# google/sentencepiece

Hardware: AMD Instinct MI355X
Metric: sentences/sec EncodeBatch, 32k unigram, MI355X (higher is better)
Workload: dtype u8 text -> i32 ids; f64 add / f32 store in the Viterbi relax

## Files before the change

### sentencepiece_amd/csrc/api.cc

```cpp
#include <hip/hip_runtime.h>

#include <cstdio>
#include <cstdlib>
#include <fcntl.h>
#include <sys/mman.h>
#include <sys/stat.h>
#include <sys/syscall.h>
#include <unistd.h>

#include <algorithm>
#include <cmath>
#include <condition_variable>
#include <cstring>
#include <fstream>
#include <functional>
#include <map>
#include <memory>
#include <mutex>
#include <thread>
#include <new>
#include <sstream>
#include <atomic>
#include <chrono>
#include <string>
// ... 135 lines not shown
      auto it = live.find(p);
      if (it == live.end()) return false;
      const size_t cap = it->second;
      live.erase(it);
      if (idle_bytes + cap > (24ull << 30)) drop = p;
      else { idle.emplace(cap, p); idle_bytes += cap; }
    }
    if (drop) (void)hipHostFree(drop);
    return true;
  }
};
PinnedPool g_pinned;

struct Profile {
  int n = 0;
  char name[kNumSlots][48] = {{0}};
  float kernel_ms[kNumSlots] = {0};
  uint64_t sentences[kNumSlots] = {0}, raw_bytes[kNumSlots] = {0}, ids[kNumSlots] = {0};
  uint64_t cycles[kNumSlots][5] = {{0}};
  uint64_t path[8] = {0};
  float total_ms = 0.f;
};

struct Workspace {
  DevBuf<uint32_t> d_lists, d_counts;
  DevBuf<uint64_t> d_tmp_off, d_tile_sums, d_chunk_base;
  DevBuf<uint32_t> d_big_list;
  DevBuf<int32_t> d_arena, d_arena_tb, d_tok_begin;
  DevBuf<uint32_t> d_span_begin, d_span_end, d_nspan_begin, d_nspan_end;
  DevBuf<uint8_t> d_norm, d_nbest_scratch, d_slab, d_pool, d_sent_status, d_flags;
  DevBuf<unsigned long long> d_res_off, d_dyn_tag;
  DevBuf<U4> d_dyn_ent, d_resume;
  DevBuf<uint32_t> d_dyn_list;
  DevBuf<float> d_res_score;
  Ctrl *d_ctrl = nullptr;
  Ctrl *h_ctrl = nullptr;
  DevBuf<uint8_t> d_text, d_dn_text;
  DevBuf<uint64_t> d_offs, d_id_offs, d_dn_offs;
  DevBuf<int32_t> d_ids;
  DevBuf<uint8_t> d_lit_bytes;
  DevBuf<uint32_t> d_lit_offs;
  DevBuf<int32_t> d_dec_ids;
  DevBuf<uint64_t> d_dec_poffs;
  const uint8_t *lit_bytes = nullptr;
  const uint32_t *lit_offs = nullptr;
  uint32_t n_lit = 0;
  PinBuf<uint8_t> h_text;
  PinBuf<uint64_t> h_offs, h_id_offs;
  uint64_t reserve_text_bytes = 0, reserve_n = 0;
  float bpe_dropout = 0.f;
  uint64_t sample_seed = 0;
  hipStream_t stream = nullptr;
  hipStream_t stream2 = nullptr;
  hipEvent_t ev_fork = nullptr, ev_join = nullptr;
  hipEvent_t ev[kNumSlots + 1][2] = {};
  bool ev_ready = false;
  bool slot_used[kNumSlots] = {false};
  char slot_name[kNumSlots][48] = {{0}};
  Profile prof;

  ~Workspace() {
    d_lists.Free(); d_counts.Free(); d_tmp_off.Free(); d_tile_sums.Free(); d_chunk_base.Free(); d_big_list.Free(); d_arena.Free();
    d_arena_tb.Free(); d_tok_begin.Free(); d_span_begin.Free(); d_span_end.Free(); d_nspan_begin.Free(); d_nspan_end.Free();
    d_norm.Free(); d_nbest_scratch.Free(); d_slab.Free(); d_pool.Free(); d_sent_status.Free(); d_flags.Free(); d_res_off.Free();
    d_res_score.Free(); d_dyn_tag.Free(); d_dyn_ent.Free(); d_dyn_list.Free(); d_resume.Free(); d_text.Free(); d_offs.Free(); d_id_offs.Free(); d_ids.Free(); d_dn_text.Free(); d_dn_offs.Free();
    h_text.Free(); h_offs.Free(); h_id_offs.Free();
// ... 27 lines not shown
  }
};
}
using spmx_tables::DevTables;

struct spmx_handle : DevTables {
  std::mutex mu;
  ModelData model;
  HostTables tables;
  std::string extra_options;
  std::string serialized;
  int device = 0;
  int n_cu = 256;
  SpmxDev dev{};
  HostTables dn_tables;
  DevBuf<uint32_t> dn_ndarts, dn_npair;
  DevBuf<uint8_t> dn_nblob;
  DevBuf<U2> dn_utrie;
  SpmxDev dn_dev{};
  std::vector<std::unique_ptr<Workspace>> pool;
  bool profiling = false;
  Profile prof;
  bool no_fast = false;
  bool no_lane_general = false;
  uint32_t char_norm_mode = 0;
  bool no_stream = false;
  uint64_t arena_first = 0;
  bool no_bp_short = false;
  bool no_wave = false;
  std::atomic<int> word_backoff{0};
  bool no_word = false;
  bool no_word_dp = false;
  uint32_t dyn_slots = kDynSlotsDefault;
  uint32_t dyn_list_cap = kDynListCapDefault;
  uint64_t nbest_budget = 32ull << 30;
  uint32_t nbest_hyps_min = 4096;
  uint32_t tile_min_lanes = 1;
  int32_t dx_npre = 0, dx_nsuf = 0, dx_pre[kMaxExtra] = {0}, dx_suf[kMaxExtra] = {0};
  bool dx_reverse = false;
  bool dx_unk = false;
  uint32_t compact_staged = 2048;
  bool no_direct = false;
  int fork_cus = 0;
  int fork_waves = 4;
  bool early_tail = false;
  bool no_overlap = false;
  bool no_ids16 = false;
  bool no_scan = false;
  bool no_word_dyn = false;
  bool memo_unsafe = false;
  bool force_word_dp = false;
  bool no_split = false;
  uint32_t split_min_raw = 576;
  bool split_own_launch = false;
  uint32_t split_tiles = 1;
  uint32_t split_per_byte = 4;
  uint32_t compact_big = kCompactBigIds;
  bool uw_exact = false;
  int uw_pipe = 1;
  bool no_uni_wave = false;
  uint32_t uni_wave_max = 0;
  int word_wgs = 1;
  uint64_t table_bytes = 0;
  uint64_t dn_table_bytes = 0;
  double load_ms = 0.0;
  int word_form = 3;
// ... 107 lines not shown
  dev->umemo16 = d->d_umemo16.p;
  dev->uall = d->d_uall.p;
  dev->udisp = d->d_udisp.p;
  dev->uhot2 = d->d_uhot2.p;
  dev->uhot = d->d_uhot.p;
  dev->pscore = d->d_pscore.p;
  dev->sym_final = d->d_sym_final.p;
  dev->sym_len = d->d_sym_len.p;
  dev->byte_ids = d->d_byte_ids.p;
  dev->dec_info = d->d_dec_info.p;
  dev->dec_off = d->d_dec_off.p;
  dev->dec_bytes = d->d_dec_bytes.p;
  return kOk;
}

int UploadDenormTables(spmx_handle *h) {
  if (!h->model.has_denormalizer) return kOk;
  const HostTables &d = h->dn_tables;
  HIP_OR_RETURN(h, Upload(&h->dn_ndarts, d.ndarts));
  HIP_OR_RETURN(h, Upload(&h->dn_nblob, d.nblob));
  HIP_OR_RETURN(h, Upload(&h->dn_npair, d.npair));
  HIP_OR_RETURN(h, Upload(&h->dn_utrie, d.utrie));
  h->dn_dev = d.scalars;
  h->dn_dev.ndarts = h->dn_ndarts.p;
  h->dn_dev.nblob = h->dn_nblob.p;
  h->dn_dev.npair = h->dn_npair.p;
  h->dn_dev.utrie = h->dn_utrie.p;
  return kOk;
}

int RefreshDevice(spmx_handle *h, bool types_changed) {
  HostTables &t = h->tables;
  if (types_changed) {
    if (h->model.model_type == kUnigram) {
      HIP_OR_RETURN(h, Upload(&h->d_ptrie, t.ptrie));
      HIP_OR_RETURN(h, Upload(&h->d_cfirst, t.cfirst));
    } else {
      HIP_OR_RETURN(h, Upload(&h->d_sym_final, t.sym_final));
    }
    HIP_OR_RETURN(h, Upload(&h->d_umemo, t.umemo));
    HIP_OR_RETURN(h, Upload(&h->d_umemo16, t.umemo16));
    HIP_OR_RETURN(h, Upload(&h->d_uall, t.uall));
    HIP_OR_RETURN(h, Upload(&h->d_udisp, t.udisp));
    HIP_OR_RETURN(h, Upload(&h->d_uhot2, t.uhot2));
    HIP_OR_RETURN(h, Upload(&h->d_uhot, t.uhot));
    HIP_OR_RETURN(h, Upload(&h->d_pscore, t.pscore));
    HIP_OR_RETURN(h, Upload(&h->d_dec_info, t.dec_info));
    HIP_OR_RETURN(h, Upload(&h->d_dec_off, t.dec_off));
    HIP_OR_RETURN(h, Upload(&h->d_dec_bytes, t.dec_bytes));
  }
  SpmxDev d = t.scalars;
  d.ndarts = h->dev.ndarts; d.nblob = h->dev.nblob; d.npair = h->dev.npair; d.ptrie = h->d_ptrie.p; d.cfirst = t.cfirst.empty() ? nullptr : h->d_cfirst.p; d.plen = h->d_plen.p; d.utrie = h->dev.utrie;
  d.chartab = h->dev.chartab; d.pairtab = h->dev.pairtab; d.wordtab = h->dev.wordtab; d.sym_final = h->d_sym_final.p;
  d.sym_len = h->dev.sym_len; d.byte_ids = h->dev.byte_ids;
  d.umemo = h->d_umemo.p; d.umemo16 = h->d_umemo16.p; d.uall = h->d_uall.p; d.udisp = h->d_udisp.p; d.uhot2 = h->d_uhot2.p; d.uhot = h->d_uhot.p; d.pscore = h->d_pscore.p;
  d.dec_info = h->d_dec_info.p; d.dec_off = h->d_dec_off.p; d.dec_bytes = h->d_dec_bytes.p;
  h->dev = d;
  return kOk;
}

void DestroyHandle(spmx_handle *h) {
  if (!h) return;
  (void)hipSetDevice(h->device);
  h->FreeTables();
  h->dn_ndarts.Free(); h->dn_npair.Free(); h->dn_nblob.Free(); h->dn_utrie.Free();
  h->pool.clear();
// ... 558 lines not shown
              sc.count = static_cast<uint32_t>(total);
              sc.tw = 64;
              sc.main_tiles = static_cast<uint32_t>((total + 63) / 64);
              sc.tile_base = 0;
              tile_base = sc.main_tiles;
            }
            continue;
          }
          if (known[c] == 0) continue;
          uint64_t tw = (static_cast<uint64_t>(known[c]) + n_waves - 1) / n_waves;
          if (tw > 64) tw = 64;
          if (tw < 1) tw = 1;
          sc.lane_shift = 6;
          sc.general = ((uni_class[c] && cls[c].rcap > kMaxStagedRaw) || cls[c].rcap > h->main_max_raw) ? 1u : 0u;
          sc.count = known[c];
          sc.tw = static_cast<uint32_t>(tw);
          sc.main_tiles = static_cast<uint32_t>((static_cast<uint64_t>(known[c]) + tw - 1) / tw);
          sc.tile_base = tile_base;
          tile_base += sc.main_tiles;
        }
        wa.total_main = tile_base;
        wa.q = &ws->d_ctrl->q[qi];
        wa.stats = &ws->d_ctrl->stats[kStatsPerClass * slot];
        wa.left_lists = out_lists;
        wa.left_counts = d_out_counts;
        wa.left2_lists = out2_lists;
        wa.left2_counts = d_out2_counts;
        wa.dyn_tag = ws->d_dyn_tag.p;
        wa.dyn_ent = ws->d_dyn_ent.p;
        wa.dyn_list = ws->d_dyn_list.p;
        wa.dyn_count = &ws->d_ctrl->dyn_count;
        wa.dyn_mask = h->dyn_slots - 1u;
        wa.dyn_cap = h->dyn_list_cap;
        wa.resume = ws->d_resume.p;
        wa.ids16 = ids16 ? 1u : 0u;
        wa.arena_first = (direct && mode != 2) ? direct_region : 0u;
        snprintf(ws->slot_name[slot], sizeof(ws->slot_name[slot]), "%s",
                 wform ? (wa.ids16 ? (mode == 2 ? "EncodeWordWaveAgainKernel<true>" : mode == 1 ? "EncodeWordWaveCollectKernel<true>" : "EncodeWordWaveKernel<true>")
                                   : (mode == 2 ? "EncodeWordWaveAgainKernel<false>" : mode == 1 ? "EncodeWordWaveCollectKernel<false>" : "EncodeWordWaveKernel<false>"))
                       : mode == 3 ? "EncodeWordDpKernel" : mode == 2 ? "EncodeWordAgainKernel" : mode == 1 ? "EncodeWordCollectKernel" : "EncodeWordKernel");
        HIP_OR_RETURN(h, record(slot, 0));
        if (wform) HIP_OR_RETURN(h, LaunchEncodeWordWave(mode, wa, static_cast<int>(grid), waves, WordWaveLdsBytes(waves), stream));
        else HIP_OR_RETURN(h, LaunchEncodeWord(mode, wa, static_cast<int>(grid), waves, WordLdsBytes(waves, dp), stream));
        HIP_OR_RETURN(h, record(slot, 1));
        ws->slot_used[slot] = true;
        return kOk;
      };
      auto read_counts = [&]() -> int {
        HIP_OR_RETURN(h, hipMemcpyAsync(ws->h_ctrl->left_counts, ws->d_ctrl->left_counts, sizeof(ws->h_ctrl->left_counts) + sizeof(uint32_t),
                                        hipMemcpyDeviceToHost, stream));
        HIP_OR_RETURN(h, hipStreamSynchronize(stream));
        return kOk;
      };
      uint64_t eligible = 0;
      for (int c = 0; c < ncls; ++c) if (cls[c].rcap <= h->main_max_raw) eligible += known[c];
      int left_at = 0;
      if (dyn) {
        FORKED_HIP_OR_RETURN(ws->d_dyn_tag.Reserve(h->dyn_slots));
        FORKED_HIP_OR_RETURN(ws->d_dyn_ent.Reserve(static_cast<size_t>(h->dyn_slots) * 4));
        FORKED_HIP_OR_RETURN(ws->d_dyn_list.Reserve(h->dyn_list_cap));
        FORKED_HIP_OR_RETURN(ws->d_resume.Reserve(n));
        FORKED_HIP_OR_RETURN(hipMemsetAsync(ws->d_dyn_tag.p, 0, static_cast<size_t>(h->dyn_slots) * sizeof(unsigned long long), stream));
        FORKED_OR_RETURN(word_pass(1, kSlotWord, 3, left_lists[0], ws->d_ctrl->left_counts[0], left_lists[1], ws->d_ctrl->left_counts[1]));
        FORKED_OR_RETURN(read_counts());
        for (int c = 0; c < ncls; ++c) { again_counts[c] = ws->h_ctrl->left_counts[0][c]; again_total += again_counts[c]; }
        again_words = ws->h_ctrl->dyn_count < h->dyn_list_cap ? ws->h_ctrl->dyn_count : h->dyn_list_cap;
        left_at = 1;
        if (again_total > 0) {
          uint32_t gone1[kMaxClasses] = {0};
          uint64_t gone1_total = 0;
          for (int c = 0; c < ncls; ++c) { gone1[c] = ws->h_ctrl->left_counts[1][c]; gone1_total += gone1[c]; }
          const bool early_tail = h->early_tail && direct && !forked && !h->no_overlap && gone1_total > 0;
          if (early_tail) {
            HIP_OR_RETURN(h, hipEventRecord(ws->ev_fork, stream));
            HIP_OR_RETURN(h, hipStreamWaitEvent(ws->stream2, ws->ev_fork, 0));
          }
          if (again_words) {
            ResolveArgs ra{};
            ra.dev = h->dev; ra.dyn_ent = ws->d_dyn_ent.p; ra.dyn_list = ws->d_dyn_list.p; ra.dyn_count = &ws->d_ctrl->dyn_count;
            ra.dyn_cap = h->dyn_list_cap; ra.unsafe = h->memo_unsafe ? 1u : 0u;
            uint64_t g = (static_cast<uint64_t>(again_words) + 63) / 64;
            if (g > static_cast<uint64_t>(h->n_cu) * 8) g = static_cast<uint64_t>(h->n_cu) * 8;
            FORKED_HIP_OR_RETURN(LaunchWordResolve(ra, static_cast<int>(g), stream));
          }
          if (early_tail) left_at = 2;
          for (int c = 0; c < ncls; ++c) known[c] = again_counts[c];
          a.lists = left_lists[0];
          FORKED_OR_RETURN(word_pass(2, kSlotWord2, 4, left_lists[left_at], ws->d_ctrl->left_counts[left_at], nullptr, nullptr));
          if (early_tail) {
            forked = true;
            stream = ws->stream2;
            tail_qi = 0;
            const int rc = general_pass(left_lists[1], ws->d_ctrl->left_counts[1], gone1, true);
            tail_qi = 5;
            hipError_t ej = rc == kOk ? hipEventRecord(ws->ev_join, stream) : hipSuccess;
            stream = main_stream;
            if (rc != kOk) return fail_forked(rc);
            if (ej != hipSuccess) return fail_forked(FailHip(h, ej, "hipEventRecord(join)"));
            a.lists = left_lists[0];
          }
          FORKED_OR_RETURN(read_counts());
        }
      } else {
        FORKED_OR_RETURN(word_pass(0, kSlotWord, 3, left_lists[0], ws->d_ctrl->left_counts[0], nullptr, nullptr));
        FORKED_OR_RETURN(read_counts());
        uint64_t total = 0;
        for (int c = 0; c < ncls; ++c) { known[c] = ws->h_ctrl->left_counts[0][c]; total += known[c]; }
        a.lists = left_lists[0];
        if (!is_bpe && !h->no_word_dp && total && (total * 4 <= n || h->force_word_dp)) {
          FORKED_OR_RETURN(word_pass(3, kSlotWord2, 4, left_lists[1], ws->d_ctrl->left_counts[1], nullptr, nullptr));
          FORKED_OR_RETURN(read_counts());
          left_at = 1;
        }
      }
      uint64_t leftover = 0;
      for (int c = 0; c < ncls; ++c) {
        known[c] = ws->h_ctrl->left_counts[left_at][c];
// ... 377 lines not shown
    if (st.ok()) st = CompileExtraOptions(h->model, "", &h->tables);
    if (st.ok() && h->model.has_denormalizer) {
      ModelData dn;
      dn.normalizer_only = true;
      dn.charsmap = h->model.dn_charsmap;
      dn.add_dummy_prefix = h->model.dn_add_dummy_prefix;
      dn.remove_extra_ws = h->model.dn_remove_extra_ws;
      dn.escape_ws = h->model.dn_escape_ws;
      st = CompileTables(dn, &h->dn_tables);
    }
    if (!st.ok()) return Fail(nullptr, st.code, st.message);
    HIP_OR_RETURN(nullptr, hipSetDevice(device));
    hipDeviceProp_t prop;
    HIP_OR_RETURN(nullptr, hipGetDeviceProperties(&prop, device));
    h->n_cu = prop.multiProcessorCount > 0 ? prop.multiProcessorCount : 256;
    for (int c = 0; c < kNumClasses; ++c) h->classes[c] = kClasses[c];
    if (const char *e = getenv("SPMX_NO_FAST")) h->no_fast = e[0] == '1';
    if (const char *e = getenv("SPMX_NO_STREAM")) h->no_stream = e[0] == '1';
    if (const char *e = getenv("SPMX_NO_WAVE")) h->no_wave = e[0] == '1';
    if (const char *e = getenv("SPMX_NO_WORD_KERNEL")) h->no_word = e[0] == '1';
    if (const char *e = getenv("SPMX_FORCE_WORD_DP")) h->force_word_dp = e[0] == '1';
    if (const char *e = getenv("SPMX_NO_WORD_DYN")) h->no_word_dyn = e[0] == '1';
    if (const char *e = getenv("SPMX_NO_OVERLAP")) h->no_overlap = e[0] == '1';
    if (const char *e = getenv("SPMX_EARLY_TAIL")) h->early_tail = e[0] == '1';
    if (const char *e = getenv("SPMX_FORK_WAVES")) h->fork_waves = atoi(e);
    if (const char *e = getenv("SPMX_FORK_CUS")) h->fork_cus = atoi(e);
    if (const char *e = getenv("SPMX_NO_DIRECT")) h->no_direct = e[0] == '1';
    if (const char *e = getenv("SPMX_COMPACT_STAGED")) {
      const long v = atol(e);
      h->compact_staged = v <= 0 ? 0u : v < 256 ? 256u : v > static_cast<long>(kCompactLdsIdsMax) ? kCompactLdsIdsMax : static_cast<uint32_t>(v) & ~7u;
    }
    if (const char *e = getenv("SPMX_NO_SCAN")) h->no_scan = e[0] == '1';
    if (const char *e = getenv("SPMX_NO_IDS16")) h->no_ids16 = e[0] == '1';
    if (const char *e = getenv("SPMX_DYN_SLOTS_LOG2")) { const int v = atoi(e); if (v >= 4 && v <= 26) h->dyn_slots = 1u << v; }
    if (const char *e = getenv("SPMX_DYN_LIST_CAP")) { const long v = atol(e); if (v >= 1 && v <= (1l << 26)) h->dyn_list_cap = static_cast<uint32_t>(v); }
    if (const char *e = getenv("SPMX_NBEST_BUDGET_GB")) { const long v = atol(e); if (v >= 1 && v <= 200) h->nbest_budget = static_cast<uint64_t>(v) << 30; }
#ifdef SPMX_TEST_SEAMS
    if (getenv("SPMX_WORDMEMO_UNSAFE")) h->memo_unsafe = true;
    if (getenv("SPMX_UW_EXACT")) h->uw_exact = true;
    if (const char *e = getenv("SPMX_COMPACT_BIG")) h->compact_big = static_cast<uint32_t>(atoll(e));
    if (const char *e = getenv("SPMX_NO_WORD_DP")) h->no_word_dp = e[0] == '1';
    if (const char *e = getenv("SPMX_NBEST_HYPS_MIN")) { const long v = atol(e); if (v >= 1024 && v <= 262144) h->nbest_hyps_min = static_cast<uint32_t>(v); }
    if (const char *e = getenv("SPMX_TILE_MIN_LANES")) h->tile_min_lanes = static_cast<uint32_t>(atoi(e));
    if (const char *e = getenv("SPMX_NO_UNI_WAVE")) h->no_uni_wave = e[0] == '1';
    if (const char *e = getenv("SPMX_WORD_WGS")) { const int v = atoi(e); if (v >= 1 && v <= 4) h->word_wgs = v; }
    if (const char *e = getenv("SPMX_NO_BP_SHORT")) h->no_bp_short = e[0] == '1';
    if (const char *e = getenv("SPMX_WIDE_TCAP")) h->wide_tcap = e[0] == '1';
    if (const char *e = getenv("SPMX_SUB_BUCKETS")) {
      const int v = atoi(e);
      h->sub_buckets = static_cast<uint32_t>(v < 1 ? 1 : (v > kMaxSubBuckets ? kMaxSubBuckets : v));
    }
    if (const char *e = getenv("SPMX_LANE_GENERAL_MIN_LANES")) h->lane_general_min_lanes = static_cast<uint32_t>(atoi(e));
    if (const char *e = getenv("SPMX_STREAM_SCRATCH_MB")) h->stream_scratch_limit = static_cast<uint64_t>(atoll(e)) << 20;
    if (const char *e = getenv("SPMX_MAIN_MAX_RAW")) h->main_max_raw = static_cast<uint32_t>(atoll(e));
    if (const char *e = getenv("SPMX_FORCE_RING")) { const int v = atoi(e); if (v >= 16 && v <= 122) h->ring_override = static_cast<uint32_t>(v); }
#else
    {
      static const char *const kSeamOnly[] = {"SPMX_NO_WORD_DP", "SPMX_NBEST_HYPS_MIN", "SPMX_TILE_MIN_LANES",
          "SPMX_NO_UNI_WAVE", "SPMX_WORD_WGS", "SPMX_NO_BP_SHORT", "SPMX_WIDE_TCAP", "SPMX_SUB_BUCKETS", "SPMX_LANE_GENERAL_MIN_LANES",
          "SPMX_STREAM_SCRATCH_MB", "SPMX_MAIN_MAX_RAW", "SPMX_FORCE_RING", "SPMX_MEMO16_ONE"};
      static std::atomic<bool> warned{false};
      for (const char *v : kSeamOnly)
        if (getenv(v) && !warned.exchange(true))
          fprintf(stderr, "libspmx: %s is read by test-seam builds only (-DSPMX_TEST_SEAMS); this library ignores it\n", v);
    }
#endif
// ... 112 lines not shown
    return RefreshDevice(h, true);
  });
}

namespace {

int RebuildForSpec(spmx_handle *h, bool add_dummy_prefix, bool remove_extra_ws, bool escape_ws, std::string *charsmap) {
  ModelData &m = h->model;
  struct Undo {
    ModelData &m;
    bool adp, rew, esc, done = false;
    std::string *charsmap;
    ~Undo() {
      if (done) return;
      m.add_dummy_prefix = adp; m.remove_extra_ws = rew; m.escape_ws = esc;
      if (charsmap) m.charsmap.swap(*charsmap);
    }
  } undo{m, m.add_dummy_prefix, m.remove_extra_ws, m.escape_ws, false, charsmap};
  m.add_dummy_prefix = add_dummy_prefix; m.remove_extra_ws = remove_extra_ws; m.escape_ws = escape_ws;
  if (charsmap) m.charsmap.swap(*charsmap);
  std::unique_ptr<HostTables> nt(new HostTables);
  Status st = CompileTables(m, nt.get());
  if (st.ok()) st = CompileExtraOptions(m, h->extra_options, nt.get());
  if (!st.ok()) return Fail(h, st.code, st.message);
  HIP_OR_RETURN(h, hipSetDevice(h->device));
  DevTables fresh;
  SpmxDev dev{};
  t_upload_bytes = 0;
  if (int rc = UploadTables(h, &fresh, *nt, &dev); rc != kOk) {
    fresh.FreeTables();
    return rc;
  }
  std::swap(static_cast<DevTables &>(*h), fresh);
  fresh.FreeTables();
  h->tables = std::move(*nt);
  h->dev = dev;
  h->table_bytes = t_upload_bytes + h->dn_table_bytes;
  h->word_backoff.store(0, std::memory_order_relaxed);
  undo.done = true;
  return kOk;
}

}

int spmx_override_normalizer_spec(spmx_handle *h, const char *const *fields, const char *const *values,
                                  const uint64_t *value_lens, uint64_t n) {
  if (!h) return kInvalidArgument;
  return Guard(h, [&]() -> int {
    if (n && (!fields || !values)) return Fail(h, kInvalidArgument, "null field or value array");
    std::vector<SpecEdit> edits;
    Status failed;
    for (uint64_t i = 0; i < n && failed.ok(); ++i) {
      const char *v = values[i] ? values[i] : "";
      SpecEdit e;
      failed = ParseSpecEdit(fields[i] ? fields[i] : "", std::string(v, value_lens ? value_lens[i] : strlen(v)), &e);
      if (failed.ok()) edits.push_back(std::move(e));
    }
    if (!edits.empty()) {
      bool adp = h->model.add_dummy_prefix, rew = h->model.remove_extra_ws, esc = h->model.escape_ws;
      const std::string *cm = nullptr;
      for (const SpecEdit &e : edits) {
        if (e.field == 2) cm = &e.bytes;
        else if (e.field == 3) adp = e.flag;
        else if (e.field == 4) rew = e.flag;
        else if (e.field == 5) esc = e.flag;
      }
// ... 1417 lines not shown
```

### sentencepiece_amd/csrc/kernels.h

```cpp
#ifndef SPMX_KERNELS_H_
#define SPMX_KERNELS_H_

#ifndef SPMX_WAVE_API
#include "wave.h"
#endif
#include <math.h>

#include "dev.h"

namespace spmx {

enum : uint32_t {
  kStArenaOverflow = 1u << 0,
  kStTooLong = 1u << 1,
  kStInternal = 1u << 2,
};
enum : uint32_t { kSsOk = 0, kSsResourceExhausted = 8, kSsOutOfRange = 11, kSsInternal = 13 };

constexpr int kMaxClasses = 8;

struct StreamClass {
  uint32_t rcap;
  uint32_t tcap;
  uint32_t lane_shift;
// ... 32 lines not shown
  uint8_t *sent_status;
  uint32_t *status;
  unsigned long long *stats;
  int32_t *arena_tb;
  uint32_t *long_list;
  SideLists *side;
  const uint32_t *lists;
  uint32_t *over_list;
  StreamQueue *q;
  uint8_t *slab;
  uint64_t slab_bytes;
  uint32_t n;
  uint32_t n_classes;
  uint32_t total_main;
  uint32_t bp_short;
  uint32_t ring;
  uint32_t fast_ok;
  uint32_t no_lane_general;
  uint32_t private_bytes;
  uint32_t split_ring;
  uint32_t match_rows;
  uint32_t no_char_norm;
  StreamClass cls[kMaxClasses];
  uint32_t *left_lists;
  uint32_t *left_counts;
  uint32_t *left2_lists;
  uint32_t *left2_counts;
  unsigned long long *dyn_tag;
  U4 *dyn_ent;
  uint32_t *dyn_list;
  uint32_t *dyn_count;
  uint32_t dyn_mask;
  uint32_t dyn_cap;
  U4 *resume;
  uint32_t ids16;
  uint32_t direct;
  uint64_t arena_first;
  const uint32_t *list;
  const uint32_t *list_count;
  uint32_t *next_list;
  uint32_t *next_count;
  uint32_t rcap, ncap;
};

constexpr int kStatsPerClass = 8;
constexpr uint32_t kTokEnd = 0x8000u;

SPMX_DEVICE uint32_t DartsOffset(uint32_t u) { return (u >> 10) << ((u & (1u << 9)) >> 6); }

SPMX_DEVICE int OneCharLenDev(uint32_t c) {
  const uint32_t h = c >> 4;
  return h < 12 ? 1 : (h < 14 ? 2 : (h == 14 ? 3 : 4));
}
SPMX_DEVICE uint32_t SpByteOf(const SpmxDev &d) { return (d.flags & kNfCompressSp) ? kSpByte : 0x100u; }

SPMX_DEVICE int wave_excl_scan(int v, int lane, int *total) {
  int incl = v;
#pragma unroll
  for (int d = 1; d < 64; d <<= 1) {
    const int up = wv::shfl_up(incl, d);
    if (lane >= d) incl += up;
  }
  *total = wv::shfl(incl, 63);
  return incl - v;
}

// ... 1094 lines not shown
```

### sentencepiece_amd/csrc/kernels_wordwave.h

```cpp
#ifndef SPMX_KERNELS_WORDWAVE_H_
#define SPMX_KERNELS_WORDWAVE_H_

namespace spmx {

constexpr uint32_t kWwRing = 4096u;
constexpr uint32_t kWwRingPad = 32u;
constexpr uint32_t kWwUnits = kWwRing / 16u;
constexpr uint32_t kWwMaskBytes = (kWwUnits + 4u) * 2u + 8u;
constexpr uint32_t kWwRecs = 128u + 512u;
constexpr uint32_t kWwMaxLen = 65536u;
constexpr uint32_t kWwPerWave = kWwRing + kWwRingPad + kWwMaskBytes + kWwRecs * 4u + 64u * 16u + 64u * 8u + 5u * 64u * 4u;
static_assert(kWwPerWave % 16u == 0u, "per-wave LDS blocks keep 16-byte alignment");
constexpr uint32_t kWwAgain = 1u, kWwGone = 2u;
constexpr uint32_t kWwKeyMaskBytes = 640u;
constexpr uint32_t kWwShared = kWwKeyMaskBytes + kWordHotSlots * 16u + kUallBuckets * 2u;
SPMX_HD constexpr bool kWwHotIn(int mode) { return mode == 2; }
SPMX_HD inline uint32_t WordWaveLdsBytes(uint32_t waves) { return kWwShared + waves * kWwPerWave; }

struct __attribute__((packed, aligned(2))) U64H { uint32_t lo, hi; };

SPMX_DEVICE uint32_t space_mask16(const Q4 &v) {
  auto m4 = [](uint32_t z) -> uint32_t { return (((z >> 7) & 0x01010101u) * 0x10204080u) >> 28; };
  return m4(space_flags(v.x)) | (m4(space_flags(v.y)) << 4) | (m4(space_flags(v.z)) << 8) | (m4(space_flags(v.w)) << 12);
}
SPMX_DEVICE uint32_t key_dword_n(uint32_t text, int n) {
  const uint32_t m = n >= 4 ? 0xFFFFFFFFu : (n <= 0 ? 0u : (1u << (8 * n)) - 1u);
  return key_dword(text, m);
}

struct WwStage {
  uint32_t cnt;
  uint32_t P, j;
  uint32_t L;
  uint32_t k0, k1, k2, k3;
  uint32_t hz, hw;
  uint32_t e0x, e0y, e0z, e0w, e1x, e1y, e1z, e1w;
  uint32_t tg_lo, tg_hi;
  uint32_t warm;
  uint32_t d0x, d0y, d0z, d0w, d1x, d1y, d1z, d1w, d2x, d2y, d2z, d2w;
};
constexpr uint32_t kWwHit16 = 0x100u;

template <int MODE, bool H16>
SPMX_DEVICE void encode_wordwave_block(const EncodeArgs &a, unsigned char *smem) {
  const int lane = wv::lane();
  const SpmxDev &d = a.dev;
  Q4 *masks = reinterpret_cast<Q4 *>(smem);
  U4 *hot = reinterpret_cast<U4 *>(smem + kWwKeyMaskBytes);
  uint16_t *disp = reinterpret_cast<uint16_t *>(smem + kWwKeyMaskBytes + kWordHotSlots * 16u);
// ... 158 lines not shown
    SA.cnt = 0u; SB.cnt = 0u;
    uint32_t carry_j = 0xFFFFFFFFu, carry_x = 0u, carry_n = 0u, carry_unk = 0u;
    uint32_t carry_t = 0u;
    unsigned long long steps = 0;

    auto stageA = [&](uint32_t qbase, uint32_t qcnt, WwStage &S) __attribute__((always_inline)) {
      S.cnt = qcnt;
      const uint32_t l32 = static_cast<uint32_t>(lane);
      const bool valid = l32 < qcnt;
      const uint32_t rec = recq[qbase + (valid ? l32 : (qcnt ? qcnt - 1u : 0u))];
      const uint32_t P = rec & 0x03FFFFFFu, j = rec >> 26;
      const uint32_t s_end = sent[j].y;
      const Q4U w = *reinterpret_cast<const Q4U *>(ring + (P & (kWwRing - 1u)));
      const U64H sm = *reinterpret_cast<const U64H *>(smask + ((P >> 4) & (kWwUnits - 1u)));
      const uint64_t bits = (static_cast<uint64_t>(sm.hi) << 32 | sm.lo) >> (P & 15u);
      const uint32_t rem = s_end - P;
      uint32_t L = static_cast<uint32_t>(wv::ffs64(bits | (1ull << 17))) - 1u;
      if (L > rem) L = rem;
      S.P = P; S.j = j;
      const Q4 mk = masks[2u * (L < 16u ? L : 16u)], pd = masks[2u * (L < 16u ? L : 16u) + 1u];
      S.k0 = (w.x & mk.x) | pd.x; S.k1 = (w.y & mk.y) | pd.y; S.k2 = (w.z & mk.z) | pd.z; S.k3 = (w.w & mk.w) | pd.w;
      const uint32_t h1 = HashWordKey(S.k0, S.k1, S.k2, S.k3), h2 = UallHash2(S.k0, S.k1, S.k2, S.k3, h1);
      const U4 e = kWwHotIn(MODE) ? hot[h1 & (kWordHotSlots - 1u)] : U4{0u, 0u, 0u, 0xFFFFFFFFu};
      const uint32_t dsp = disp[UallBucket(h2)];
      const uint32_t zmask = L <= 10u ? 0xFFFFu : 0xFFFFFFFFu, form = L <= 10u ? kMemo16TwoPiece : 0u;
      const bool hit16 = kWwHotIn(MODE) & (valid & (L <= 12u)) & ((e.x == S.k0) & (e.y == S.k1)) & ((((e.z ^ S.k2) & zmask) == 0u) &
                         ((e.w & kMemo16TwoPiece) == form) & (e.w != 0xFFFFFFFFu));
      S.L = L | (hit16 ? kWwHit16 : 0u);
      S.hz = e.z; S.hw = e.w;
      const uint32_t slp = perfect ? UallSlot(h1, h2, dsp, mall) : (h1 & mall);
      const uint32_t sl = (valid & !hit16 & (L <= 16u)) ? slp : 0u;
      const U4 e0 = uall[2u * sl], e1 = uall[2u * sl + 1u];
      S.e0x = e0.x; S.e0y = e0.y; S.e0z = e0.z; S.e0w = e0.w; S.e1x = e1.x; S.e1y = e1.y; S.e1z = e1.z; S.e1w = e1.w;
      if (MODE != kWmPlain) {
        const bool pre = MODE == kWmDyn || dyn_warm != 0u;
        if (MODE == kWmCollect && dyn_warm != 0u) --dyn_warm;
        const uint32_t dsl = (pre & valid & !hit16 & (L <= 16u)) ? (h1 & a.dyn_mask) : 0u;
        const unsigned long long g = MODE == kWmCollect ? wv::atomic_load64(&a.dyn_tag[dsl]) : a.dyn_tag[dsl];
        S.tg_lo = static_cast<uint32_t>(g); S.tg_hi = static_cast<uint32_t>(g >> 32);
        S.warm = pre ? 1u : 0u;
        if (MODE == kWmDyn) {
          const U4 d0 = a.dyn_ent[4u * dsl], d1 = a.dyn_ent[4u * dsl + 1u], d2 = a.dyn_ent[4u * dsl + 2u];
          S.d0x = d0.x; S.d0y = d0.y; S.d0z = d0.z; S.d0w = d0.w; S.d1x = d1.x; S.d1y = d1.y; S.d1z = d1.z; S.d1w = d1.w;
          S.d2x = d2.x; S.d2y = d2.y; S.d2z = d2.z; S.d2w = d2.w;
        }
      }
    };
    auto stageB = [&](WwStage &S) __attribute__((always_inline)) {
      if (S.cnt == 0u) return;
      ++steps;
      const bool word = static_cast<uint32_t>(lane) < S.cnt;
      const uint32_t k0 = S.k0, k1 = S.k1, k2 = S.k2, k3 = S.k3, j = S.j, P = S.P;
      const bool lng = (S.L & 0xFFu) > 16u;
      const bool hit16 = kWwHotIn(MODE) && (S.L & kWwHit16) != 0u;
      const bool probe = word && !hit16 && !lng;
      U4 e0{S.e0x, S.e0y, S.e0z, S.e0w}, e1{S.e1x, S.e1y, S.e1z, S.e1w};
      bool hit32 = probe & ((e0.x == k0) & (e0.y == k1)) & ((e0.z == k2) & (e0.w == k3)) & (e1.x != 0xFFFFFFFFu);
      bool walk = !perfect && probe && !hit32 && e1.x != 0xFFFFFFFFu;
      if (wv::any(walk)) {
        uint32_t sl = HashWordKey(k0, k1, k2, k3) & mall;
        while (wv::any(walk)) {
          ++tc.cyc[1];
          if (walk) {
            sl = (sl + 1u) & mall;
            e0 = uall[2u * sl];
            e1 = uall[2u * sl + 1u];
            hit32 = e0.x == k0 && e0.y == k1 && e0.z == k2 && e0.w == k3 && e1.x != 0xFFFFFFFFu;
            walk = !hit32 && e1.x != 0xFFFFFFFFu;
          }
        }
      }
      bool hitd = false;
      uint32_t dn = 0;
      U4 dia{0, 0, 0, 0}, dib{0, 0, 0, 0};
      uint32_t dbound = 0u, dlim = 0u;
      if (MODE == kWmDyn && wv::any(probe & !hit32)) {
        if (probe & !hit32) {
          const unsigned long long tag = DynTag(k0, k1, k2, k3);
          uint32_t sl = static_cast<uint32_t>(tag >> 32) & a.dyn_mask;
          unsigned long long g = static_cast<unsigned long long>(S.tg_hi) << 32 | S.tg_lo;
          U4 d0{S.d0x, S.d0y, S.d0z, S.d0w}, d1{S.d1x, S.d1y, S.d1z, S.d1w}, d2{S.d2x, S.d2y, S.d2z, S.d2w};
          for (uint32_t t = 0; t < kDynProbes; ++t) {
            if (g == 0ull) break;
            if (g == tag) {
              if (d0.x == k0 && d0.y == k1 && d0.z == k2 && d0.w == k3 && d1.x == 1u) {
                hitd = true; dn = d1.y; dbound = d1.z; dlim = d1.w;
                dia = d2;
                const uint32_t cn = d1.y & 0xFFu;
                if ((d1.y & kDynWide) ? cn > 8u : cn > 4u) dib = a.dyn_ent[4u * sl + 3u];
              }
              break;
            }
            sl = (sl + 1u) & a.dyn_mask;
            g = a.dyn_tag[sl];
            d0 = a.dyn_ent[4u * sl]; d1 = a.dyn_ent[4u * sl + 1u]; d2 = a.dyn_ent[4u * sl + 2u];
          }
        }
      }
      const bool hit = hit16 || hit32 || hitd;
      bool gone = word && lng;
      bool miss = false;
      if (MODE == kWmCollect) {
        if (wv::any(probe && !hit32)) {
          dyn_warm = 16u;
          if (probe && !hit32) {
            auto plain = [](uint32_t v) -> bool {
              return (((v + 0x01010101u) | v) & 0x80808080u) == 0u && (((v - 0x20202020u) & ~v) & 0x80808080u) == 0u;
            };
            bool kept = false;
            if (any_word || (plain(k0) && plain(k1) && plain(k2) && plain(k3))) {
              const unsigned long long tag = DynTag(k0, k1, k2, k3);
              uint32_t sl = static_cast<uint32_t>(tag >> 32) & a.dyn_mask;
              unsigned long long g0 = static_cast<unsigned long long>(S.tg_hi) << 32 | S.tg_lo;
              const bool have0 = S.warm != 0u;
              for (uint32_t t = 0; t < kDynProbes && !kept; ++t) {
                unsigned long long g = (t == 0u && have0) ? g0 : wv::atomic_load64(&a.dyn_tag[sl]);
                if (g == 0ull) g = wv::atomic_cas(&a.dyn_tag[sl], 0ull, tag);
                if (g == 0ull) {
                  const uint32_t at2 = wv::atomic_add(a.dyn_count, 1u);
                  a.dyn_ent[4u * sl] = U4{k0, k1, k2, k3};
                  a.dyn_ent[4u * sl + 1u] = U4{at2 < a.dyn_cap ? 0u : 2u, 0u, 0u, 0u};
                  if (at2 < a.dyn_cap) { a.dyn_list[at2] = sl; kept = true; }
                  break;
                }
                if (g == tag) { kept = true; break; }
                sl = (sl + 1u) & a.dyn_mask;
              }
            }
            if (kept) miss = true; else gone = true;
          }
        }
      } else {
        if (probe && !hit) gone = true;
      }
      uint32_t id0, id1, x;
      float lim;
      if (hit16) {
        id0 = S.hw & 0xFFFFu;
        id1 = ((S.hw & kMemo16TwoPiece) && (S.hz >> 16) != 0xFFFFu) ? S.hz >> 16 : 0xFFFFFFFFu;
        x = S.hw >> 24;
        lim = wv::bits_to_float((((S.hw >> 16) & 0x7Fu) + 127u) << 23);
      } else {
        id0 = e1.x; id1 = e1.y;
        const float xf = wv::bits_to_float(hitd ? dbound : e1.z);
        x = xf < 8192.f ? static_cast<uint32_t>(xf) : 8192u;
        lim = wv::bits_to_float(hitd ? dlim : e1.w);
      }
      if (!hit) x = 0u;
      if (hit && x >= 8192u) { gone = true; x = 0u; }
      const uint32_t jprev = wv::lane_up1(j, 0xFFFFFFFFu);
      const bool head = jprev != j;
      const uint32_t j0 = wv::read_lane(j, 0);
      const bool cont = j == j0 && j0 == carry_j;
      uint32_t skip = 0u;
      const uint32_t lastunk = (word && hitd && (dn & kDynLastUnk)) ? 1u : 0u;
      if (MODE == kWmDyn) {
        const uint32_t pl = wv::lane_up1(lastunk, 0u);
        const bool prev_unk = head ? (cont && carry_unk != 0u) : pl != 0u;
        if (hitd && (dn & kDynFirstUnk) && prev_unk) skip = 1u;
      }
      const uint32_t cntd = dn & 0xFFu;
      if (MODE == kWmDyn) {
        const uint32_t pl = wv::lane_up1(lastunk, 0u);
        const bool prev_unk = head ? (cont && carry_unk != 0u) : pl != 0u;
        if (word && hitd && cntd == 0u && prev_unk) gone = true;
      }
      const uint32_t cnt = !word ? 0u : (hitd ? cntd - skip : (hit ? (id1 != 0xFFFFFFFFu ? 2u : 1u) : 0u));
      const uint32_t packed = (x << 12) | cnt;
      const uint32_t Sc = wv::scan_add(packed);
      const uint32_t E = Sc - packed;
      const uint32_t T = carry_t + (E & 0xFFFu);
      carry_t += wv::read_lane(Sc, 63) & 0xFFFu;
      const uint32_t hE = wv::scan_max(head ? E : 0u);
      const uint32_t rel = E - hE;
      uint32_t xb = rel >> 12, nb = rel & 0xFFFu;
      uint32_t n0j = 0u;
      if (MODE == kWmDyn) n0j = s_n0[j];
      if (cont) { xb += carry_x; nb += carry_n; }
      else if (MODE == kWmDyn) { xb += s_x0[j]; nb += n0j; }
      {
        const int lv = static_cast<int>(S.cnt - 1u);
        carry_j = wv::read_lane(j, lv);
        carry_x = wv::read_lane(xb + x, lv);
        carry_n = wv::read_lane(nb + cnt, lv);
        carry_unk = wv::read_lane(lastunk, lv);
      }
      if (word && hit && !(xb < (1u << 24) && static_cast<float>(xb) < lim)) gone = true;
      const U4 sj = sent[j];
      if (MODE == kWmDyn && word && hit && nb + cnt > sj.y - sj.x + 1u + n0j) gone = true;
      const uint64_t so = (static_cast<uint64_t>(sj.w) << 32 | sj.z) + T;
      if (word && hit && so + cnt > rend) gone = true;
      const bool emit = word && hit && !gone;
      if (emit && !hitd) {
        if (H16) {
          uint16_t *q = reinterpret_cast<uint16_t *>(a.arena) + so;
          q[0] = static_cast<uint16_t>(id0);
          if (cnt == 2u) q[1] = static_cast<uint16_t>(id1);
        } else {
          int32_t *q = a.arena + so;
          q[0] = static_cast<int32_t>(id0);
          if (cnt == 2u) q[1] = static_cast<int32_t>(id1);
        }
      }
      if (MODE == kWmDyn && wv::any(emit && hitd)) {
        const bool wide = (dn & kDynWide) != 0u;
        auto idc = [&](uint32_t t) __attribute__((always_inline)) -> uint32_t {
          const uint32_t di[8] = {dia.x, dia.y, dia.z, dia.w, dib.x, dib.y, dib.z, dib.w};
          if (wide) return t < 16u ? (di[(t >> 1) & 7u] >> (16u * (t & 1u))) & 0xFFFFu : 0u;
          return t < 8u ? di[t & 7u] : 0u;
        };
        const uint32_t maxc = wv::read_lane(wv::scan_max((emit && hitd) ? cnt : 0u), 63);
#pragma unroll
        for (uint32_t t = 0; t < kDynMaxWide; ++t) {
          if (t >= maxc) break;
          if (emit && hitd && t < cnt) {
            const uint32_t id = skip ? idc(t + 1u) : idc(t);
            if (H16) reinterpret_cast<uint16_t *>(a.arena)[so + t] = static_cast<uint16_t>(id);
            else a.arena[so + t] = static_cast<int32_t>(id);
          }
        }
      }
      const uint32_t jnext = wv::lane_down1(word ? j : 0xFFFFFFFEu, 0xFFFFFFFEu);
      if (word && jnext != j) s_nids[j] = nb + cnt;
      if (wv::any(gone || miss)) {
        if (gone) wv::lds_atomic_or(&s_stat[j], kWwGone);
        if (miss) { wv::lds_atomic_or(&s_stat[j], kWwAgain); wv::lds_atomic_min(&s_first[j], P); }
        wv::sync();
        if (MODE == kWmCollect) {
          const bool wr = miss && s_first[j] == P;
          const uint32_t sidj = wv::shfl(sid, static_cast<int>(j));
          if (wr) a.resume[sidj] = U4{P - sj.x, nb, wv::float_to_bits(static_cast<float>(xb)), 0u};
        }
      }
    };
    auto tick2 = [&](uint32_t qbase, uint32_t q1, uint32_t q2) __attribute__((always_inline)) {
      stageA(qbase, q1, SA);
      stageB(SB);
      stageA(qbase + 64u, q2, SB);
// ... 159 lines not shown
```

Measured before the change: 2.389 billion.

## Carry the dynamic word memo table across EncodeBatch calls

```diff
diff --git a/sentencepiece_amd/csrc/api.cc b/sentencepiece_amd/csrc/api.cc
--- a/sentencepiece_amd/csrc/api.cc
+++ b/sentencepiece_amd/csrc/api.cc
@@ -191,6 +191,10 @@
   DevBuf<unsigned long long> d_res_off, d_dyn_tag;
   DevBuf<U4> d_dyn_ent, d_resume;
   DevBuf<uint32_t> d_dyn_list;
+  const void *dyn_made_at = nullptr;
+  uint32_t dyn_made_slots = 0;
+  uint64_t dyn_epoch = 0, dyn_live = 0;
+  bool dyn_dirty = false;
   DevBuf<float> d_res_score;
   Ctrl *d_ctrl = nullptr;
   Ctrl *h_ctrl = nullptr;
@@ -284,6 +288,8 @@
   bool no_word = false;
   bool no_word_dp = false;
   uint32_t dyn_slots = kDynSlotsDefault;
+  bool dyn_carry = true;
+  std::atomic<uint64_t> memo_epoch{1};
   uint32_t dyn_list_cap = kDynListCapDefault;
   uint64_t nbest_budget = 32ull << 30;
   uint32_t nbest_hyps_min = 4096;
@@ -457,6 +463,7 @@
 int RefreshDevice(spmx_handle *h, bool types_changed) {
   HostTables &t = h->tables;
   if (types_changed) {
+    h->memo_epoch.fetch_add(1, std::memory_order_relaxed);
     if (h->model.model_type == kUnigram) {
       HIP_OR_RETURN(h, Upload(&h->d_ptrie, t.ptrie));
       HIP_OR_RETURN(h, Upload(&h->d_cfirst, t.cfirst));
@@ -1081,6 +1088,7 @@
         wa.dyn_count = &ws->d_ctrl->dyn_count;
         wa.dyn_mask = h->dyn_slots - 1u;
         wa.dyn_cap = h->dyn_list_cap;
+        wa.dyn_look = h->dyn_carry ? 1u : 0u;
         wa.resume = ws->d_resume.p;
         wa.ids16 = ids16 ? 1u : 0u;
         wa.arena_first = (direct && mode != 2) ? direct_region : 0u;
@@ -1109,12 +1117,38 @@
         FORKED_HIP_OR_RETURN(ws->d_dyn_ent.Reserve(static_cast<size_t>(h->dyn_slots) * 4));
         FORKED_HIP_OR_RETURN(ws->d_dyn_list.Reserve(h->dyn_list_cap));
         FORKED_HIP_OR_RETURN(ws->d_resume.Reserve(n));
-        FORKED_HIP_OR_RETURN(hipMemsetAsync(ws->d_dyn_tag.p, 0, static_cast<size_t>(h->dyn_slots) * sizeof(unsigned long long), stream));
+        const uint64_t epoch = h->memo_epoch.load(std::memory_order_relaxed);
+        const bool fresh = ws->dyn_made_at != ws->d_dyn_tag.p || ws->dyn_made_slots != h->dyn_slots || ws->dyn_epoch != epoch ||
+                           ws->dyn_live * 2 > h->dyn_slots || ws->dyn_dirty;
+        if (!h->dyn_carry || fresh) {
+          FORKED_HIP_OR_RETURN(hipMemsetAsync(ws->d_dyn_tag.p, 0, static_cast<size_t>(h->dyn_slots) * sizeof(unsigned long long), stream));
+          if (h->dyn_carry) FORKED_HIP_OR_RETURN(hipMemsetAsync(ws->d_dyn_ent.p, 0, static_cast<size_t>(h->dyn_slots) * 4 * sizeof(U4), stream));
+          ws->dyn_made_at = h->dyn_carry ? ws->d_dyn_tag.p : nullptr;
+          ws->dyn_made_slots = h->dyn_slots;
+          ws->dyn_epoch = epoch;
+          ws->dyn_live = 0;
+        }
+        ws->dyn_dirty = true;
         FORKED_OR_RETURN(word_pass(1, kSlotWord, 3, left_lists[0], ws->d_ctrl->left_counts[0], left_lists[1], ws->d_ctrl->left_counts[1]));
         FORKED_OR_RETURN(read_counts());
         for (int c = 0; c < ncls; ++c) { again_counts[c] = ws->h_ctrl->left_counts[0][c]; again_total += again_counts[c]; }
         again_words = ws->h_ctrl->dyn_count < h->dyn_list_cap ? ws->h_ctrl->dyn_count : h->dyn_list_cap;
+        ws->dyn_live += ws->h_ctrl->dyn_count;
         left_at = 1;
+        auto resolve_words = [&]() -> hipError_t {
+          if (again_words) {
+            ResolveArgs ra{};
+            ra.dev = h->dev; ra.dyn_ent = ws->d_dyn_ent.p; ra.dyn_list = ws->d_dyn_list.p; ra.dyn_count = &ws->d_ctrl->dyn_count;
+            ra.dyn_cap = h->dyn_list_cap; ra.unsafe = h->memo_unsafe ? 1u : 0u;
+            uint64_t g = (static_cast<uint64_t>(again_words) + 63) / 64;
+            if (g > static_cast<uint64_t>(h->n_cu) * 8) g = static_cast<uint64_t>(h->n_cu) * 8;
+            hipError_t e = LaunchWordResolve(ra, static_cast<int>(g), stream);
+            if (e != hipSuccess) return e;
+          }
+          ws->dyn_dirty = false;
+          return hipSuccess;
+        };
+        if (again_total == 0 && h->dyn_carry) FORKED_HIP_OR_RETURN(resolve_words());
         if (again_total > 0) {
           uint32_t gone1[kMaxClasses] = {0};
           uint64_t gone1_total = 0;
@@ -1124,14 +1158,7 @@
             HIP_OR_RETURN(h, hipEventRecord(ws->ev_fork, stream));
             HIP_OR_RETURN(h, hipStreamWaitEvent(ws->stream2, ws->ev_fork, 0));
           }
-          if (again_words) {
-            ResolveArgs ra{};
-            ra.dev = h->dev; ra.dyn_ent = ws->d_dyn_ent.p; ra.dyn_list = ws->d_dyn_list.p; ra.dyn_count = &ws->d_ctrl->dyn_count;
-            ra.dyn_cap = h->dyn_list_cap; ra.unsafe = h->memo_unsafe ? 1u : 0u;
-            uint64_t g = (static_cast<uint64_t>(again_words) + 63) / 64;
-            if (g > static_cast<uint64_t>(h->n_cu) * 8) g = static_cast<uint64_t>(h->n_cu) * 8;
-            FORKED_HIP_OR_RETURN(LaunchWordResolve(ra, static_cast<int>(g), stream));
-          }
+          FORKED_HIP_OR_RETURN(resolve_words());
           if (early_tail) left_at = 2;
           for (int c = 0; c < ncls; ++c) known[c] = again_counts[c];
           a.lists = left_lists[0];
@@ -1575,6 +1602,7 @@
     }
     if (const char *e = getenv("SPMX_NO_SCAN")) h->no_scan = e[0] == '1';
     if (const char *e = getenv("SPMX_NO_IDS16")) h->no_ids16 = e[0] == '1';
+    if (const char *e = getenv("SPMX_DYN_CARRY")) h->dyn_carry = e[0] != '0';
     if (const char *e = getenv("SPMX_DYN_SLOTS_LOG2")) { const int v = atoi(e); if (v >= 4 && v <= 26) h->dyn_slots = 1u << v; }
     if (const char *e = getenv("SPMX_DYN_LIST_CAP")) { const long v = atol(e); if (v >= 1 && v <= (1l << 26)) h->dyn_list_cap = static_cast<uint32_t>(v); }
     if (const char *e = getenv("SPMX_NBEST_BUDGET_GB")) { const long v = atol(e); if (v >= 1 && v <= 200) h->nbest_budget = static_cast<uint64_t>(v) << 30; }
@@ -1753,6 +1781,7 @@
     return rc;
   }
   std::swap(static_cast<DevTables &>(*h), fresh);
+  h->memo_epoch.fetch_add(1, std::memory_order_relaxed);
   fresh.FreeTables();
   h->tables = std::move(*nt);
   h->dev = dev;
diff --git a/sentencepiece_amd/csrc/kernels.h b/sentencepiece_amd/csrc/kernels.h
--- a/sentencepiece_amd/csrc/kernels.h
+++ b/sentencepiece_amd/csrc/kernels.h
@@ -88,6 +88,7 @@
   uint32_t *dyn_count;
   uint32_t dyn_mask;
   uint32_t dyn_cap;
+  uint32_t dyn_look;
   U4 *resume;
   uint32_t ids16;
   uint32_t direct;
diff --git a/sentencepiece_amd/csrc/kernels_wordwave.h b/sentencepiece_amd/csrc/kernels_wordwave.h
--- a/sentencepiece_amd/csrc/kernels_wordwave.h
+++ b/sentencepiece_amd/csrc/kernels_wordwave.h
@@ -15,6 +15,7 @@
 constexpr uint32_t kWwKeyMaskBytes = 640u;
 constexpr uint32_t kWwShared = kWwKeyMaskBytes + kWordHotSlots * 16u + kUallBuckets * 2u;
 SPMX_HD constexpr bool kWwHotIn(int mode) { return mode == 2; }
+SPMX_HD constexpr bool kWwDynIn(int mode) { return mode != 0; }
 SPMX_HD inline uint32_t WordWaveLdsBytes(uint32_t waves) { return kWwShared + waves * kWwPerWave; }
 
 struct __attribute__((packed, aligned(2))) U64H { uint32_t lo, hi; };
@@ -239,7 +240,7 @@
       const uint32_t sl = (valid & !hit16 & (L <= 16u)) ? slp : 0u;
       const U4 e0 = uall[2u * sl], e1 = uall[2u * sl + 1u];
       S.e0x = e0.x; S.e0y = e0.y; S.e0z = e0.z; S.e0w = e0.w; S.e1x = e1.x; S.e1y = e1.y; S.e1z = e1.z; S.e1w = e1.w;
-      if (MODE != kWmPlain) {
+      if (kWwDynIn(MODE)) {
         const bool pre = MODE == kWmDyn || dyn_warm != 0u;
         if (MODE == kWmCollect && dyn_warm != 0u) --dyn_warm;
         const uint32_t dsl = (pre & valid & !hit16 & (L <= 16u)) ? (h1 & a.dyn_mask) : 0u;
@@ -277,30 +278,51 @@
           }
         }
       }
-      bool hitd = false;
+      bool hitd = false, dfound = false, ddead = false;
       uint32_t dn = 0;
       U4 dia{0, 0, 0, 0}, dib{0, 0, 0, 0};
       uint32_t dbound = 0u, dlim = 0u;
-      if (MODE == kWmDyn && wv::any(probe & !hit32)) {
-        if (probe & !hit32) {
-          const unsigned long long tag = DynTag(k0, k1, k2, k3);
-          uint32_t sl = static_cast<uint32_t>(tag >> 32) & a.dyn_mask;
-          unsigned long long g = static_cast<unsigned long long>(S.tg_hi) << 32 | S.tg_lo;
-          U4 d0{S.d0x, S.d0y, S.d0z, S.d0w}, d1{S.d1x, S.d1y, S.d1z, S.d1w}, d2{S.d2x, S.d2y, S.d2z, S.d2w};
-          for (uint32_t t = 0; t < kDynProbes; ++t) {
-            if (g == 0ull) break;
-            if (g == tag) {
-              if (d0.x == k0 && d0.y == k1 && d0.z == k2 && d0.w == k3 && d1.x == 1u) {
+      const bool ask = probe & !hit32;
+      auto plain = [](uint32_t v) -> bool {
+        return (((v + 0x01010101u) | v) & 0x80808080u) == 0u && (((v - 0x20202020u) & ~v) & 0x80808080u) == 0u;
+      };
+      const bool look = ask && (MODE != kWmCollect || any_word || (plain(k0) && plain(k1) && plain(k2) && plain(k3)));
+      unsigned long long dtag = 0ull, dg = 0ull;
+      uint32_t dsl = 0u, dt = 0u;
+      if (kWwDynIn(MODE) && wv::any(look)) {
+        if (look) {
+          dtag = DynTag(k0, k1, k2, k3);
+          dsl = static_cast<uint32_t>(dtag >> 32) & a.dyn_mask;
+          dg = static_cast<unsigned long long>(S.tg_hi) << 32 | S.tg_lo;
+          U4 d0{0, 0, 0, 0}, d1{0, 0, 0, 0}, d2{0, 0, 0, 0};
+          if (MODE == kWmDyn) { d0 = U4{S.d0x, S.d0y, S.d0z, S.d0w}; d1 = U4{S.d1x, S.d1y, S.d1z, S.d1w}; d2 = U4{S.d2x, S.d2y, S.d2z, S.d2w}; }
+          if (MODE == kWmCollect) {
+            const bool have_tag = S.warm != 0u;
+            if (!have_tag) dg = wv::atomic_load64(&a.dyn_tag[dsl]);
+            if (!have_tag || dg != 0ull) { d0 = a.dyn_ent[4u * dsl]; d1 = a.dyn_ent[4u * dsl + 1u]; }
+          }
+          const bool usable = MODE == kWmDyn || a.dyn_look != 0u;
+          for (; dt < kDynProbes; ++dt) {
+            if (dg == 0ull) break;
+            if (dg == dtag) {
+              dfound = true;
+              const bool same = d0.x == k0 && d0.y == k1 && d0.z == k2 && d0.w == k3;
+              if (same && d1.x == 1u && usable) {
                 hitd = true; dn = d1.y; dbound = d1.z; dlim = d1.w;
-                dia = d2;
-                const uint32_t cn = d1.y & 0xFFu;
-                if ((d1.y & kDynWide) ? cn > 8u : cn > 4u) dib = a.dyn_ent[4u * sl + 3u];
+                if (MODE == kWmDyn) {
+                  dia = d2;
+                  const uint32_t cn = d1.y & 0xFFu;
+                  if ((d1.y & kDynWide) ? cn > 8u : cn > 4u) dib = a.dyn_ent[4u * dsl + 3u];
+                }
+              } else if (same && d1.x == 2u && usable) {
+                ddead = true;
               }
               break;
             }
-            sl = (sl + 1u) & a.dyn_mask;
-            g = a.dyn_tag[sl];
-            d0 = a.dyn_ent[4u * sl]; d1 = a.dyn_ent[4u * sl + 1u]; d2 = a.dyn_ent[4u * sl + 2u];
+            dsl = (dsl + 1u) & a.dyn_mask;
+            dg = MODE == kWmCollect ? wv::atomic_load64(&a.dyn_tag[dsl]) : a.dyn_tag[dsl];
+            d0 = a.dyn_ent[4u * dsl]; d1 = a.dyn_ent[4u * dsl + 1u];
+            if (MODE == kWmDyn) d2 = a.dyn_ent[4u * dsl + 2u];
           }
         }
       }
@@ -308,30 +330,23 @@
       bool gone = word && lng;
       bool miss = false;
       if (MODE == kWmCollect) {
-        if (wv::any(probe && !hit32)) {
+        if (wv::any(ask)) {
           dyn_warm = 16u;
-          if (probe && !hit32) {
-            auto plain = [](uint32_t v) -> bool {
-              return (((v + 0x01010101u) | v) & 0x80808080u) == 0u && (((v - 0x20202020u) & ~v) & 0x80808080u) == 0u;
-            };
-            bool kept = false;
-            if (any_word || (plain(k0) && plain(k1) && plain(k2) && plain(k3))) {
-              const unsigned long long tag = DynTag(k0, k1, k2, k3);
-              uint32_t sl = static_cast<uint32_t>(tag >> 32) & a.dyn_mask;
-              unsigned long long g0 = static_cast<unsigned long long>(S.tg_hi) << 32 | S.tg_lo;
-              const bool have0 = S.warm != 0u;
-              for (uint32_t t = 0; t < kDynProbes && !kept; ++t) {
-                unsigned long long g = (t == 0u && have0) ? g0 : wv::atomic_load64(&a.dyn_tag[sl]);
-                if (g == 0ull) g = wv::atomic_cas(&a.dyn_tag[sl], 0ull, tag);
-                if (g == 0ull) {
+          if (ask && !hitd) {
+            bool kept = dfound && !ddead;
+            if (look && !dfound) {
+              for (; dt < kDynProbes && !kept; ++dt) {
+                if (dg == 0ull) dg = wv::atomic_cas(&a.dyn_tag[dsl], 0ull, dtag);
+                if (dg == 0ull) {
                   const uint32_t at2 = wv::atomic_add(a.dyn_count, 1u);
-                  a.dyn_ent[4u * sl] = U4{k0, k1, k2, k3};
-                  a.dyn_ent[4u * sl + 1u] = U4{at2 < a.dyn_cap ? 0u : 2u, 0u, 0u, 0u};
-                  if (at2 < a.dyn_cap) { a.dyn_list[at2] = sl; kept = true; }
+                  a.dyn_ent[4u * dsl] = U4{k0, k1, k2, k3};
+                  a.dyn_ent[4u * dsl + 1u] = U4{at2 < a.dyn_cap ? 0u : 2u, 0u, 0u, 0u};
+                  if (at2 < a.dyn_cap) { a.dyn_list[at2] = dsl; kept = true; }
                   break;
                 }
-                if (g == tag) { kept = true; break; }
-                sl = (sl + 1u) & a.dyn_mask;
+                if (dg == dtag) { kept = true; break; }
+                dsl = (dsl + 1u) & a.dyn_mask;
+                dg = wv::atomic_load64(&a.dyn_tag[dsl]);
               }
             }
             if (kept) miss = true; else gone = true;
@@ -361,16 +376,13 @@
       const bool cont = j == j0 && j0 == carry_j;
       uint32_t skip = 0u;
       const uint32_t lastunk = (word && hitd && (dn & kDynLastUnk)) ? 1u : 0u;
-      if (MODE == kWmDyn) {
+      const uint32_t cntd = dn & 0xFFu;
+      if (kWwDynIn(MODE)) {
         const uint32_t pl = wv::lane_up1(lastunk, 0u);
         const bool prev_unk = head ? (cont && carry_unk != 0u) : pl != 0u;
         if (hitd && (dn & kDynFirstUnk) && prev_unk) skip = 1u;
-      }
-      const uint32_t cntd = dn & 0xFFu;
-      if (MODE == kWmDyn) {
-        const uint32_t pl = wv::lane_up1(lastunk, 0u);
-        const bool prev_unk = head ? (cont && carry_unk != 0u) : pl != 0u;
         if (word && hitd && cntd == 0u && prev_unk) gone = true;
+        if (MODE == kWmCollect && miss && prev_unk) { miss = false; gone = true; }
       }
       const uint32_t cnt = !word ? 0u : (hitd ? cntd - skip : (hit ? (id1 != 0xFFFFFFFFu ? 2u : 1u) : 0u));
       const uint32_t packed = (x << 12) | cnt;
@@ -394,7 +406,7 @@
       }
       if (word && hit && !(xb < (1u << 24) && static_cast<float>(xb) < lim)) gone = true;
       const U4 sj = sent[j];
-      if (MODE == kWmDyn && word && hit && nb + cnt > sj.y - sj.x + 1u + n0j) gone = true;
+      if (kWwDynIn(MODE) && word && hit && nb + cnt > sj.y - sj.x + 1u + n0j) gone = true;
       const uint64_t so = (static_cast<uint64_t>(sj.w) << 32 | sj.z) + T;
       if (word && hit && so + cnt > rend) gone = true;
       const bool emit = word && hit && !gone;
@@ -409,8 +421,12 @@
           if (cnt == 2u) q[1] = static_cast<int32_t>(id1);
         }
       }
-      if (MODE == kWmDyn && wv::any(emit && hitd)) {
+      if (kWwDynIn(MODE) && wv::any(emit && hitd)) {
         const bool wide = (dn & kDynWide) != 0u;
+        if (MODE == kWmCollect && emit && hitd) {
+          dia = a.dyn_ent[4u * dsl + 2u];
+          if (wide ? cntd > 8u : cntd > 4u) dib = a.dyn_ent[4u * dsl + 3u];
+        }
         auto idc = [&](uint32_t t) __attribute__((always_inline)) -> uint32_t {
           const uint32_t di[8] = {dia.x, dia.y, dia.z, dia.w, dib.x, dib.y, dib.z, dib.w};
           if (wide) return t < 16u ? (di[(t >> 1) & 7u] >> (16u * (t & 1u))) & 0xFFFFu : 0u;
```

Result: faster. 2.524 billion, median of 6 (+5.7%).
